# jingsenzhu/i2-sdf

Measured on AMD Instinct MI355X. Metric: ray-samples/sec (fwd+bwd), higher is better.
Workload: dtype f32 (bf16x3 split MFMA: fp32 operands as 3 bf16 terms, fp32 accumulate; the 256x256 weight-gradient GEMM blocks and the sampler's depth-choosing sdf-only passes: 2 bf16 terms per operand, 3 products, fp32 accumulate; the saved SDF tensors abar / G(hbar) / G(a) -- operands of those GEMMs and of the s

## Files before the change

### i2sdf_amd/csrc/mlp_args.h

```cpp
#pragma once
#include "mlp_common.h"

struct SdfTrainFwdArgs {
  const float* fwd; int n_fwd;
  const float* rev; int n_rev;
  int L, skip;
  i2sdf::PointSpec pts;
  int64_t M, Mp;
  float* sdf;
  float* feat;
  float* grad;
  float* hs;
  float* abars;
  float* pe_save;
  int kcs = 16;
  int p24 = 0;
  int wg0 = 0;
  int64_t ldf = 0;
};

struct SdfBwdArgs {
  const float* fwd; int n_fwd;
  const float* rev; int n_rev;
  int L, skip;
// ... 11 lines not shown
  int kcs = 16;
  int p24 = 0;
  int wg0 = 0;
};

struct RgbFwdArgs {
  const float* fwd; int n_fwd; int L;
  const float* dirs; int n_per_ray;
  const float* feat;
  int64_t M, Mp;
  float* rgb;
  float* rs;
  float* pev_save;
  int kcs = 16;
  int wg0 = 0;
};

struct RgbBwdArgs {
  const float* rev; int n_rev; int L;
  int64_t M, Mp;
  const float* rgb;
  const float* rgb_bar;
  const float* rs;
  float* gar;
  float* ga_last;
  float* fbar;
  int kcs = 16;
  int wg0 = 0;
};

void i2sdf_launch_igrad3(const SdfTrainFwdArgs& a, unsigned grid, hipStream_t st);
void i2sdf_launch_sdf_bwd3(const SdfBwdArgs& a, unsigned grid, hipStream_t st);
void i2sdf_launch_train_fwd3h(const SdfTrainFwdArgs& a, unsigned grid, hipStream_t st);
void i2sdf_launch_rgb_fwd3h(const RgbFwdArgs& a, unsigned grid, hipStream_t st);
void i2sdf_launch_rgb_bwd3h(const RgbBwdArgs& a, unsigned grid, hipStream_t st);
struct LightFwd3hArgs {
  const float* fwd; int n_fwd;
  const float* feat;
  int64_t M;
  float* lm;
  float* hl;
};
void i2sdf_launch_light_fwd3h(const LightFwd3hArgs& a, unsigned grid, hipStream_t st);
// ... 1 lines not shown
```

### i2sdf_amd/csrc/mlp_bwd.hip

```cpp
#include "ksplit.h"
#include "mlp_args.h"

using namespace i2sdf;

int i2sdf_hip_check(hipError_t e, const char* what);


namespace {

template <int H, int F, int LF>
__global__ __launch_bounds__(256) void sdf_bwd_kernel(SdfBwdArgs a) {
  constexpr int NT = H / 32, KC = H / 8, PEC = PE<LF>::PEC, PT = cdiv(PEC * 8, 32), FC = F / 8;
  extern __shared__ __attribute__((aligned(16))) float lds[];
  const int tid = threadIdx.x, lane = tid & 63, wave = tid >> 6, hi = lane >> 5;
  const int64_t m = ((int64_t)(blockIdx.x + a.wg0) * 4 + wave) * 32 + (lane & 31);
  const bool valid = m < a.M;
  const int64_t mc = valid ? m : a.M - 1;
  const int64_t lstride = a.Mp * H;
  float gp[PEC * 4];
  {
    float px, py, pz, full[PEC * 8], coef[PEC * 8], nb[3] = {0.f, 0.f, 0.f};
    fetch_point(a.pts, mc, px, py, pz);
    pe_full<LF>(px, py, pz, full);
    pe_coef<LF>(full, coef);
// ... 347 lines not shown
    auto full = [&](hipStream_t s, int wg0, unsigned g, int64_t Mv) {
      SdfBwdArgs x = x3 ? a3 : a;
      x.wg0 = wg0; x.M = Mv;
      if (x3) i2sdf_launch_sdf_bwd3(x, g, s);
      else launch_lds(sdf_bwd_kernel<256, 256, 6>, g, s, x);
    };
    i2sdf_dispatch_points(p, st, M, ranged, true, TAIL_FORKED, full, tail);
  } else if (p->H == 64 && p->F == 64) {
    launch_lds(sdf_bwd_kernel<64, 64, 6>, (unsigned)((M + PTS_PER_WG - 1) / PTS_PER_WG), st, a);
  } else return I2SDF_EINVAL;
  return i2sdf_hip_check(hipGetLastError(), "sdf_backward launch");
}

extern "C" int i2sdf_rgb_backward(const i2sdf_plan* p, const float* packed, const float* rgb, const float* rgb_bar, const float* rs,
                                  int64_t M, int64_t Mp, float* gar, float* ga_last, float* fbar, void* stream) {
  if (M == 0) return I2SDF_OK;
  if (!p || !packed || !rgb || !rgb_bar || !rs || !gar || !ga_last || !fbar || M < 0) return I2SDF_EINVAL;
  if (Mp < M || Mp % PTS_PER_WG) return I2SDF_EINVAL;
  const i2sdf_mlp_desc& d = p->rgb.d;
  const bool wide = d.hidden == 256 && p->F == 256, x3 = wide && p->rgb_bf16x3;
  if (!wide && !(d.hidden == 64 && p->F == 64)) return I2SDF_EINVAL;
  const Span rev = span(p, packed, p->rgb, SPAN_REV);
  if (!rev.n_stages) return I2SDF_EINVAL;
  RgbBwdArgs a{};
  a.rev = rev.w; a.n_rev = rev.n_stages;
  a.L = d.n_lin; a.M = M; a.Mp = Mp; a.rgb = rgb; a.rgb_bar = rgb_bar; a.rs = rs; a.gar = gar; a.ga_last = ga_last; a.fbar = fbar;
  RgbBwdArgs a3 = a;
  if (x3) {
    const Span rev3 = span(p, packed, p->rgb, SPAN_REV3H);
    if (!rev3.n_stages) return I2SDF_EINVAL;
    a3.rev = rev3.w; a3.n_rev = rev3.n_stages;
    a3.kcs = rgb_blocked_points(p, M, Mp) > 0 ? KCS_BLK : KCS_PM;
  }
  hipStream_t st = (hipStream_t)stream;
  const bool ranged = x3 && i2sdf_parts_on(p);
  ChainGuard guard(p, st, ranged);
  auto full = [&](hipStream_t s, int wg0, unsigned g, int64_t Mv) {
    RgbBwdArgs x = x3 ? a3 : a;
    x.wg0 = wg0; x.M = Mv;
    if (x3) i2sdf_launch_rgb_bwd3h(x, g, s);
    else launch_lds(rgb_bwd_kernel<256, 256>, g, s, x);
  };
  auto tail = [&](hipStream_t s, int64_t m0) {
    launch_lds_bytes(KS_LDS_BYTES, rgb_bwd_split_kernel<256, 256>, (unsigned)((M - m0 + 31) / 32), s, a, m0);
  };
  if (wide) i2sdf_dispatch_points(p, st, M, ranged, true, TAIL_BEHIND, full, tail);
  else launch_lds(rgb_bwd_kernel<64, 64>, (unsigned)((M + PTS_PER_WG - 1) / PTS_PER_WG), st, a);
// ... 3 lines not shown
```

### i2sdf_amd/csrc/mlp_train.hip

```cpp
#include "ksplit.h"
#include "mlp_args.h"

using namespace i2sdf;

int i2sdf_hip_check(hipError_t e, const char* what);


namespace {

template <int H, int F, int LF, bool GRAD>
__global__ __launch_bounds__(256) void sdf_train_fwd_kernel(SdfTrainFwdArgs a) {
  constexpr int NT = H / 32, KC = H / 8, PEC = PE<LF>::PEC, PT = cdiv(PEC * 8, 32), FT = F / 32;
  extern __shared__ __attribute__((aligned(16))) float lds[];
  const int tid = threadIdx.x, lane = tid & 63, wave = tid >> 6, hi = lane >> 5;
  const int64_t m = ((int64_t)(blockIdx.x + a.wg0) * 4 + wave) * 32 + (lane & 31);
  const bool valid = m < a.M;
  const int64_t mc = valid ? m : a.M - 1;
  float px, py, pz;
  fetch_point(a.pts, mc, px, py, pz);
  float pe[PEC * 4];
  {
    float full[PEC * 8];
    pe_full<LF>(px, py, pz, full);
    to_b_layout<PEC>(full, pe, hi);
// ... 353 lines not shown
      if (grad) i2sdf_launch_igrad3(x, g, s);
    } else if (wide) {
      if (grad) launch_lds(sdf_train_fwd_kernel<256, 256, 6, true>, g, s, x);
      else launch_lds(sdf_train_fwd_kernel<256, 256, 6, false>, g, s, x);
    } else {
      if (grad) launch_lds(sdf_train_fwd_kernel<64, 64, 6, true>, g, s, x);
      else launch_lds(sdf_train_fwd_kernel<64, 64, 6, false>, g, s, x);
    }
  };
  i2sdf_dispatch_points(p, st, M, ranged, wide && feat != nullptr, TAIL_FORKED, full, tail);
  return i2sdf_hip_check(hipGetLastError(), "sdf_forward_grad launch");
}

extern "C" int i2sdf_rgb_forward(const i2sdf_plan* p, const float* packed, const float* dirs, int32_t n_per_ray, const float* feat,
                                 int64_t M, int64_t Mp, float* rgb, float* rs, float* pev_save, void* stream) {
  if (M == 0) return I2SDF_OK;
  if (!p || !packed || !dirs || !feat || !rgb || M < 0 || n_per_ray <= 0) return I2SDF_EINVAL;
  if (Mp < M || Mp % PTS_PER_WG) return I2SDF_EINVAL;
  const i2sdf_mlp_desc& d = p->rgb.d;
  if (d.multires != 4) return I2SDF_EINVAL;
  const bool wide = d.hidden == 256 && p->F == 256, x3 = wide && p->rgb_bf16x3;
  if (!wide && !(d.hidden == 64 && p->F == 64)) return I2SDF_EINVAL;
  const Span fwd = span(p, packed, p->rgb, SPAN_FWD);
  if (!fwd.n_stages) return I2SDF_EINVAL;
  RgbFwdArgs a{};
  a.fwd = fwd.w; a.n_fwd = fwd.n_stages;
  a.L = d.n_lin; a.dirs = dirs; a.n_per_ray = n_per_ray; a.feat = feat; a.M = M; a.Mp = Mp; a.rgb = rgb; a.rs = rs; a.pev_save = pev_save;
  RgbFwdArgs a3 = a;
  if (x3) {
    const Span fwd3 = span(p, packed, p->rgb, SPAN_FWD3H);
    if (!fwd3.n_stages) return I2SDF_EINVAL;
    a3.fwd = fwd3.w; a3.n_fwd = fwd3.n_stages;
    a3.kcs = rgb_blocked_points(p, M, Mp) > 0 ? KCS_BLK : KCS_PM;
  }
  hipStream_t st = (hipStream_t)stream;
  const bool ranged = x3 && i2sdf_parts_on(p);
  ChainGuard guard(p, st, ranged);
  auto full = [&](hipStream_t s, int wg0, unsigned g, int64_t Mv) {
    RgbFwdArgs x = x3 ? a3 : a;
    x.wg0 = wg0; x.M = Mv;
    if (x3) i2sdf_launch_rgb_fwd3h(x, g, s);
    else launch_lds(rgb_fwd_kernel<256, 256, 4>, g, s, x);
  };
  auto tail = [&](hipStream_t s, int64_t m0) {
    launch_lds_bytes(KS_LDS_BYTES, rgb_fwd_split_kernel<256, 256, 4>, (unsigned)((M - m0 + 31) / 32), s, a, m0);
  };
  if (wide) i2sdf_dispatch_points(p, st, M, ranged, true, TAIL_BEHIND, full, tail);
  else launch_lds(rgb_fwd_kernel<64, 64, 4>, (unsigned)((M + PTS_PER_WG - 1) / PTS_PER_WG), st, a);
// ... 112 lines not shown
```

### i2sdf_amd/csrc/mlp_x3h.hip

```cpp
#define I2SDF_RELU_ASM 1
#include "mlp_args.h"
#include "x3h.h"

using namespace i2sdf;

namespace {

template <int LF>
__device__ __forceinline__ void pe_select_h(float px, float py, float pz, float (&pe)[cdiv(PE<LF>::DIM, 32) * 8], int kg) {
  constexpr int PED = PE<LF>::DIM, PE32 = cdiv(PED, 32);
  float full[PE<LF>::PEC * 8], pad[PE32 * 32];
  pe_full<LF>(px, py, pz, full);
#pragma unroll
  for (int i = 0; i < PE32 * 32; ++i) pad[i] = (i < PED) ? full[i < PE<LF>::PEC * 8 ? i : 0] : 0.f;
  x3h_select<PE32>(pad, pe, kg);
}

template <int H, int LF, int NW, int PL>
__global__ __launch_bounds__(NW * 64, 2) void sdf_fwd3h_kernel(const float* __restrict__ stream, int n_stages, int L, int skip, PointSpec ps,
                                                                const int* __restrict__ skip_flag, int64_t M, float* __restrict__ sdf_out) {
  constexpr int NT = H / 16, KH32 = H / 32, PE32 = cdiv(PE<LF>::DIM, 32), NPE = PE32 * 8;
  extern __shared__ __attribute__((aligned(16))) float lds[];
  if (skip_flag != nullptr && skip_flag[0] != 0) return;
  const int tid = threadIdx.x, lane = tid & 63, wave = tid >> 6, kg = lane >> 4;
// ... 77 lines not shown
#pragma unroll
    for (int r = 0; r < 4; ++r) h[nt * 4 + r] = softplus100(accA[nt][r]);
  if (a.hs) store_regs_h<NT>(a.hs + (a.L - 2) * lstride + mrow, kg, valid, h, kcs);
  {
    float s[1];
    rowvec_h<1, NT, NW>(ws, h, s, tid);
    if (a.sdf != nullptr && valid && kg == 0) a.sdf[m] = s[0];
  }
  if (a.feat != nullptr) {
    XhRegSrc<NT * 4> src{h};
    dense_x3h<FT, KH32, 1, NW>(ws, src, accB, tid);
    store_tile_h<FT>(a.feat + mc * (a.ldf ? a.ldf : (int64_t)F), kg, valid, accB);
  }
}

template <int H, int F, int LFV, int NW>
__global__ __launch_bounds__(NW * 64, 2) void rgb_fwd3h_kernel(RgbFwdArgs a) {
  constexpr int NT = H / 16, KH32 = H / 32, PECV = PE<LFV>::PEC, PV32 = cdiv(PE<LFV>::DIM, 32);
  extern __shared__ __attribute__((aligned(16))) float lds[];
  const int tid = threadIdx.x, lane = tid & 63, wave = tid >> 6, kg = lane >> 4;
  const int64_t m = ((int64_t)(blockIdx.x + a.wg0) * NW + wave) * HP + (lane & 15);
  const bool valid = m < a.M;
  const int64_t mc = valid ? m : a.M - 1;
  const int64_t ray = mc / a.n_per_ray;
  float pev[PV32 * 8];
  pe_select_h<LFV>(a.dirs[ray * 3 + 0], a.dirs[ray * 3 + 1], a.dirs[ray * 3 + 2], pev, kg);
  if (a.pev_save) store_pe_row_h<PECV>(a.pev_save + m * (PECV * 8), kg, valid, pev);
  const int64_t lstride = a.Mp * H;
  const int kcs = a.kcs;
  const int64_t mrow = save_row_off(m, kcs);
  WStreamH<NW> ws;
  ws.begin(a.fwd, lds, a.n_fwd, tid);
  f32x4 accA[NT], accB[NT];
  {
    XhPeRowSrc<PV32> src{pev, a.feat + mc * F, kg};
    dense_x3h<NT, PV32 + F / 32, 1, NW>(ws, src, accA, tid);
  }
  for (int l = 1; l < a.L - 1; ++l) {
    XhReluSrc<NT> src{accA, a.rs ? a.rs + (l - 1) * lstride + mrow : nullptr, kg, valid, kcs};
    dense_x3h<NT, KH32, 1, NW>(ws, src, accB, tid);
#pragma unroll
    for (int nt = 0; nt < NT; ++nt) accA[nt] = accB[nt];
  }
  float r[NT * 4];
#pragma unroll
  for (int nt = 0; nt < NT; ++nt)
#pragma unroll
    for (int q = 0; q < 4; ++q) r[nt * 4 + q] = fmaxf(accA[nt][q], 0.f);
  if (a.rs) store_regs_h<NT>(a.rs + (a.L - 2) * lstride + mrow, kg, valid, r, kcs);
  float o[3];
  rowvec_h<3, NT, NW>(ws, r, o, tid);
  if (valid && kg == 0) {
#pragma unroll
    for (int i = 0; i < 3; ++i) a.rgb[m * 3 + i] = 1.0f / (1.0f + expf(-o[i]));
  }
}

template <int HL, int F, int NW>
__global__ __launch_bounds__(NW * 64, 2) void light_fwd3h_kernel(LightFwd3hArgs a) {
  constexpr int NT = HL / 16, KF32 = F / 32;
  extern __shared__ __attribute__((aligned(16))) float lds[];
  const int tid = threadIdx.x, lane = tid & 63, wave = tid >> 6, kg = lane >> 4;
  const int64_t m = ((int64_t)blockIdx.x * NW + wave) * HP + (lane & 15);
  const bool valid = m < a.M;
// ... 4 lines not shown
  {
    XhRowSrc<true> src{a.feat + mc * F, kg};
    dense_x3h<NT, KF32, 1, NW>(ws, src, acc, tid);
  }
  float h[NT * 4];
#pragma unroll
  for (int nt = 0; nt < NT; ++nt)
#pragma unroll
    for (int r = 0; r < 4; ++r) h[nt * 4 + r] = softplus100(acc[nt][r]);
  if (a.hl) store_regs_h<NT>(a.hl + m * HL, kg, valid, h, 16);
  float o[1];
  rowvec_h<1, NT, NW>(ws, h, o, tid);
  if (valid && kg == 0) a.lm[m] = 1.0f / (1.0f + expf(-o[0]));
}

template <int H, int F, int NW>
__global__ __launch_bounds__(NW * 64, 2) void rgb_bwd3h_kernel(RgbBwdArgs a) {
  constexpr int NT = H / 16, KH32 = H / 32, FT = F / 16;
  static_assert(FT == NT, "feature tiles reuse the hidden accumulator set");
  extern __shared__ __attribute__((aligned(16))) float lds[];
  const int tid = threadIdx.x, lane = tid & 63, wave = tid >> 6, kg = lane >> 4;
  const int64_t m = ((int64_t)(blockIdx.x + a.wg0) * NW + wave) * HP + (lane & 15);
  const bool valid = m < a.M;
  const int64_t mc = valid ? m : a.M - 1;
  const int64_t lstride = a.Mp * H;
  const int kcs = a.kcs;
  const int64_t mrow = save_row_off(m, kcs), mcrow = save_row_off(mc, kcs);
  float g3[3];
#pragma unroll
  for (int j = 0; j < 3; ++j) {
    const float c = a.rgb[mc * 3 + j];
    g3[j] = a.rgb_bar[mc * 3 + j] * c * (1.0f - c);
  }
  if (valid && kg == 0) *reinterpret_cast<f32x4*>(a.ga_last + m * 4) = f32x4{g3[0], g3[1], g3[2], 0.f};
  WStreamH<NW> ws;
  ws.begin(a.rev, lds, a.n_rev, tid);
  float ga[NT * 4];
  {
    constexpr int NWC = 3 * NT, TOT = rowvec_h_chunks(NT, 3), NS = TOT / SCH;
#pragma unroll
    for (int i = 0; i < NT * 4; ++i) ga[i] = 0.f;
#pragma unroll
    for (int s = 0; s < NS; ++s) {
      const f32x4* cur = reinterpret_cast<const f32x4*>(ws.advance(tid)) + lane;
#pragma unroll
      for (int j = 0; j < SCH; ++j) {
        const int c = s * SCH + j;
        if (c < NWC) {
          const int row = c / NT, nt = c % NT;
          const f32x4 w = cur[j * 64];
          ga[nt * 4 + 0] = fmaf(w.x, g3[row], ga[nt * 4 + 0]);
          ga[nt * 4 + 1] = fmaf(w.y, g3[row], ga[nt * 4 + 1]);
          ga[nt * 4 + 2] = fmaf(w.z, g3[row], ga[nt * 4 + 2]);
          ga[nt * 4 + 3] = fmaf(w.w, g3[row], ga[nt * 4 + 3]);
        }
      }
    }
    const int l = a.L - 2;
    const float* rrow = a.rs + l * lstride + mcrow;
    float* grow = a.gar + l * lstride + mrow;
#pragma unroll
    for (int nt = 0; nt < NT; ++nt) {
      const f32x4 rv = *reinterpret_cast<const f32x4*>(rrow + nt * kcs + 4 * kg);
      f32x4 o;
#pragma unroll
      for (int t = 0; t < 4; ++t) { o[t] = rv[t] > 0.f ? ga[nt * 4 + t] : 0.f; ga[nt * 4 + t] = o[t]; }
      if (valid) *reinterpret_cast<f32x4*>(grow + nt * kcs + 4 * kg) = o;
    }
  }
  f32x4 accA[NT], accB[NT];
  auto zero = [&](f32x4 (&x)[NT]) __attribute__((always_inline)) {
#pragma unroll
    for (int nt = 0; nt < NT; ++nt) x[nt] = f32x4{0.f, 0.f, 0.f, 0.f};
  };
  {
    XhRegSrc<NT * 4> src{ga};
    zero(accA);
    dense_x3h<NT, KH32, 0, NW>(ws, src, accA, tid);
  }
  for (int l = a.L - 3; l >= 1; --l) {
    XhMaskSrc<NT> src{accA, a.rs + l * lstride + mcrow, a.gar + l * lstride + mrow, kg, valid, kcs};
    zero(accB);
    dense_x3h<NT, KH32, 0, NW>(ws, src, accB, tid);
#pragma unroll
    for (int nt = 0; nt < NT; ++nt) accA[nt] = accB[nt];
  }
  {
    XhMaskSrc<NT> src{accA, a.rs + mcrow, a.gar + mrow, kg, valid, kcs};
    zero(accB);
    dense_x3h<FT, KH32, 0, NW>(ws, src, accB, tid);
    store_tile_h<FT>(a.fbar + mc * F, kg, valid, accB);
  }
}

}

void i2sdf_launch_sdf_fwd3h(const float* stream, int n_stages, int L, int skip, const PointSpec& ps, const int* skip_flag, int64_t M, float* sdf_out,
                            int planes, hipStream_t st) {
  const unsigned grid = (unsigned)((M + 8 * HP - 1) / (8 * HP));
  if (planes == 2) launch_lds_threads(512, sdf_fwd3h_kernel<256, 6, 8, 2>, grid, st, stream, n_stages, L, skip, ps, skip_flag, M, sdf_out);
  else launch_lds_threads(512, sdf_fwd3h_kernel<256, 6, 8, 3>, grid, st, stream, n_stages, L, skip, ps, skip_flag, M, sdf_out);
}
void i2sdf_launch_train_fwd3h(const SdfTrainFwdArgs& a, unsigned grid, hipStream_t st) { launch_lds_threads(512, sdf_train_fwd3h_kernel<256, 256, 6, 8>, grid, st, a); }
void i2sdf_launch_rgb_fwd3h(const RgbFwdArgs& a, unsigned grid, hipStream_t st) { launch_lds_threads(512, rgb_fwd3h_kernel<256, 256, 4, 8>, grid, st, a); }
void i2sdf_launch_light_fwd3h(const LightFwd3hArgs& a, unsigned grid, hipStream_t st) { launch_lds_threads(8 * 64, light_fwd3h_kernel<128, 256, 8>, grid, st, a); }
void i2sdf_launch_rgb_bwd3h(const RgbBwdArgs& a, unsigned grid, hipStream_t st) { launch_lds_threads(512, rgb_bwd3h_kernel<256, 256, 8>, grid, st, a); }
```

### i2sdf_amd/csrc/x3h.h

```cpp
#pragma once
#include "x3.h"

namespace i2sdf {

constexpr int HP = 16;
constexpr int XH_AHEAD = 1, XH_RING = XH_AHEAD + 1;
constexpr int SCH = SC;
constexpr int LDS_BYTES_H = LDS_BYTES;
template <int NW> using WStreamH = WStreamT<NW * 64, SCH>;

__host__ __device__ constexpr int x3h_op_chunks(int NT, int KC32, int PL = 3) { return round_up(NT + KC32 * NT * PL, SCH); }
__host__ __device__ constexpr int x3h_bwd_chunks(int KT, int KC32) { return round_up(KC32 * KT * 3, SCH); }
__host__ __device__ constexpr int rowvec_h_chunks(int NTK, int nrows) { return round_up(nrows * NTK + 1, SCH); }

__device__ __forceinline__ f32x4 mfma_bf16h(u32x4 a, u32x4 b, f32x4 c) {
  return __builtin_amdgcn_mfma_f32_16x16x32_bf16(__builtin_bit_cast(bf16x8, a), __builtin_bit_cast(bf16x8, b), c, 0, 0, 0);
}

template <int NC32>
__device__ __forceinline__ void x3h_select(const float (&full)[NC32 * 32], float (&sel)[NC32 * 8], int kg) {
  const unsigned m1 = (kg & 1) ? 0xffffffffu : 0u, m2 = (kg & 2) ? 0xffffffffu : 0u;
  auto pick = [](unsigned m, float a, float b) __attribute__((always_inline)) {
    return __builtin_bit_cast(float, (__builtin_bit_cast(unsigned, a) & m) | (__builtin_bit_cast(unsigned, b) & ~m));
  };
// ... 204 lines not shown
    if (kc < KACC && hrow != nullptr && valid) x3h_store8(hrow, kc, kg, v, kcs);
    return 0;
  }
};
template <int NREG>
struct XhRegSrc {
  static constexpr bool STORES = false;
  const float (&r)[NREG];
  __device__ __forceinline__ int ahead(int) { return 0; }
  __device__ __forceinline__ float p1(int, int) { return 0.f; }
  __device__ __forceinline__ float p2(int, int, float) { return 0.f; }
  __device__ __forceinline__ float p3(int kc, int u, float, float, float&) { return r[8 * kc + u]; }
  __device__ __forceinline__ int done(int, const float (&)[8], const float (&)[8]) { return 0; }
};

template <int NT>
struct XhReluSrc {
  static constexpr bool STORES = true;
  const f32x4 (&accP)[NT]; float* rrow; int kg; bool valid; int kcs = 16;
  __device__ __forceinline__ int ahead(int) { return 0; }
  __device__ __forceinline__ float p1(int, int) { return 0.f; }
  __device__ __forceinline__ float p2(int, int, float) { return 0.f; }
  __device__ __forceinline__ float p3(int kc, int u, float, float, float&) { return relu0(accP[2 * kc + (u >> 2)][u & 3]); }
  __device__ __forceinline__ int done(int kc, const float (&v)[8], const float (&)[8]) {
    if (rrow != nullptr && valid) x3h_store8(rrow, kc, kg, v, kcs);
    return 0;
  }
};
template <int NPV>
struct XhPeRowSrc {
  static constexpr bool STORES = false;
  const float (&pe)[NPV * 8]; const float* row; int kg;
  f32x4 q[XH_RING][2];
  __device__ __forceinline__ int ahead(int kc) { if (kc >= NPV) x3h_load8(row, kc - NPV, kg, q[kc % XH_RING], 16); return kc >= NPV ? 2 : 0; }
  __device__ __forceinline__ float p1(int, int) { return 0.f; }
  __device__ __forceinline__ float p2(int, int, float) { return 0.f; }
  __device__ __forceinline__ float p3(int kc, int u, float, float, float&) { return kc < NPV ? pe[8 * (kc < NPV ? kc : 0) + u] : q[kc % XH_RING][u >> 2][u & 3]; }
  __device__ __forceinline__ int done(int, const float (&)[8], const float (&)[8]) { return 0; }
// ... 14 lines not shown
};
template <int NT>
struct XhMaskSrc {
  static constexpr bool STORES = true;
  const f32x4 (&accP)[NT]; const float* rrow; float* grow; int kg; bool valid; int kcs = 16;
  f32x4 q[XH_RING][2];
  __device__ __forceinline__ int ahead(int kc) { x3h_load8(rrow, kc, kg, q[kc % XH_RING], kcs); return 2; }
  __device__ __forceinline__ float p1(int, int) { return 0.f; }
  __device__ __forceinline__ float p2(int, int, float) { return 0.f; }
  __device__ __forceinline__ float p3(int kc, int u, float, float, float&) { return q[kc % XH_RING][u >> 2][u & 3] > 0.f ? accP[2 * kc + (u >> 2)][u & 3] : 0.f; }
  __device__ __forceinline__ int done(int kc, const float (&v)[8], const float (&)[8]) {
    x3h_store8(grow, kc, kg, v, kcs);
    return X3_COUNT_STORES ? 2 : 0;
  }
};

template <int NTK>
__device__ __forceinline__ void store_regs_h(float* __restrict__ row, int kg, bool valid, const float (&r)[NTK * 4], int kcs) {
  if (!valid) return;
#pragma unroll
  for (int nt = 0; nt < NTK; ++nt) stg4(row + nt * kcs + 4 * kg, f32x4{r[4 * nt], r[4 * nt + 1], r[4 * nt + 2], r[4 * nt + 3]});
}
template <int NTK>
__device__ __forceinline__ void store_tile_h(float* __restrict__ row, int kg, bool valid, const f32x4 (&t)[NTK]) {
  if (!valid) return;
#pragma unroll
  for (int nt = 0; nt < NTK; ++nt) stg4(row + 16 * nt + 4 * kg, t[nt]);
}
}
```

### i2sdf_amd/engine.py

```python
from __future__ import annotations

import ctypes as C
from typing import Optional

import os

import torch

from . import lib as L
from .config import NetConfig
from .params import ParamLayout


class RenderEngine:
    def __init__(self, cfg: NetConfig, device="cuda"):
        self.cfg = cfg
        self.layout = ParamLayout(cfg)
        self.device = torch.device(device)
        self._lib = L.load()
        self._desc = self.layout.net_desc()
        plan = C.c_void_p()
        L.check(self._lib.i2sdf_plan_create(C.byref(self._desc), C.byref(plan)), "i2sdf_plan_create")
        self._plan = plan
        self.pack_floats = int(self._lib.i2sdf_plan_pack_floats(plan))
        self.wgrad_floats = int(self._lib.i2sdf_plan_wgrad_floats(plan))
        self.packed = torch.zeros(self.pack_floats, dtype=torch.float32, device=self.device)
        self._pack_stream, self._pack_event, self._pack_readers = None, None, {}
        self.F = cfg.feature_size
        wide = cfg.sdf.hidden == 256 and cfg.feature_size == 256
        self.set_sdf_forward_bf16x3(bool(cfg.bf16x3 and cfg.sdf.hidden % 64 == 0))
        self.set_wgrad_bf16x3(bool(cfg.bf16x3))
        self.set_train_forward_bf16x3(bool(cfg.bf16x3 and wide))
        self.set_sdf_backward_bf16x3(bool(cfg.bf16x3 and wide))
        self.set_rgb_bf16x3(bool(cfg.bf16x3 and cfg.rgb.hidden == 256 and cfg.feature_size == 256 and cfg.rgb.n_lin >= 3))
        self.wgrad_bf16x2 = False
        x2 = os.environ.get("I2SDF_WGRAD_BF16X2", "")
        self.set_wgrad_bf16x2(bool(cfg.bf16x3 and ((x2 != "0") if x2 != "" else cfg.wgrad_bf16x2)))
        self.sampler_bf16x2 = False
        sx2 = os.environ.get("I2SDF_SAMPLER_BF16X2", "")
        if wide:
            self.set_sampler_bf16x2(bool(self.sdf_forward_bf16x3 and ((sx2 != "0") if sx2 != "" else getattr(cfg, "sampler_bf16x2", False))))
        self.set_blocked_saves(bool(cfg.bf16x3 and os.environ.get("I2SDF_BLOCKED_SAVES", "1") != "0"))
        self.saves24 = False
        s24 = os.environ.get("I2SDF_SAVES24", "")
        if wide:
            self.set_saves24(bool(cfg.bf16x3 and ((s24 != "0") if s24 != "" else getattr(cfg, "saves24", True))))
        self.set_tail_overlap(os.environ.get("I2SDF_TAIL_OVERLAP", "1") != "0")
        self.parts = 0
        n_parts = int(os.environ.get("I2SDF_PARTS", "2"))
# ... 7 lines not shown
        self.u_more = torch.linspace(0.0, 1.0, steps=sc.N_samples_eval, device=dev)
        self.u_final = torch.linspace(0.0, 1.0, steps=sc.N_samples, device=dev)
        if sc.N_samples_extra > 0:
            self.extra_tab = torch.stack([torch.linspace(0, sc.N_samples_eval * (it + 1) - 1, sc.N_samples_extra).long()
                                          for it in range(sc.max_total_iters)]).to(torch.int32).to(dev).contiguous()
        else:
            self.extra_tab = None
        self.n_z = sc.N_samples + sc.N_samples_extra + 2

    def start_timing(self):
        self._timing = []
        eng = self

        class _Timed:
            def __init__(self, fn, name):
                self.fn, self.name = fn, name

            def __call__(self, *a):
                e0, e1 = torch.cuda.Event(enable_timing=True), torch.cuda.Event(enable_timing=True)
                e0.record()
                rc = self.fn(*a)
                e1.record()
                eng._timing.append((self.name, e0, e1))
                return rc

        self._timed_lib = type("TimedLib", (), {})()
        for name in L.SIGNATURES:
            fn = getattr(self._lib, name)
            if name in ("i2sdf_sdf_forward", "i2sdf_sdf_forward_grad", "i2sdf_rgb_forward", "i2sdf_rgb_backward", "i2sdf_sdf_backward",
                        "i2sdf_weight_grads", "i2sdf_sample_rays", "i2sdf_composite_forward", "i2sdf_composite_backward", "i2sdf_pack_weights",
                        "i2sdf_ray_setup", "i2sdf_light_forward", "i2sdf_light_backward"):
                fn = _Timed(fn, name)
            setattr(self._timed_lib, name, fn)
        self._real_lib, self._lib = self._lib, self._timed_lib

    def stop_timing(self):
        self._lib = self._real_lib
        out = {}
        for name, e0, e1 in self._timing:
            tot, cnt = out.get(name, (0.0, 0))
            out[name] = (tot + e0.elapsed_time(e1), cnt + 1)
        self._timing = []
        return out

# ... 105 lines not shown
                out[l] = v.reshape(Mp, 256)
        return out

    def saved_pm(self, name: str, t: torch.Tensor, M: int, has_feat: bool = True) -> torch.Tensor:
        Mp = t.shape[1]
        if name in ("rs", "gar"):
            return self.saved_to_point_major(t, self.blocked_points(1, M, Mp))[:, :M]
        nb = self.blocked_points(0, M, Mp, has_feat)
        p24 = None
        if name in ("abars", "gus", "gas") and self.saves24_points(M, Mp, has_feat) == Mp:
            p24 = [True] * t.shape[0]
            if name == "gus":
                p24[-1] = False
                p24[0] = False
        return self.saved_to_point_major(t, nb, p24)[:, :M]

    def set_tail_overlap(self, on: bool):
        L.check(self._lib.i2sdf_plan_set_option(self._plan, L.OPT_TAIL_OVERLAP, int(bool(on))), "i2sdf_plan_set_option")
        self.tail_overlap = bool(on)

    def _sync_parts(self):
        want = self._parts_wanted if (self.train_forward_bf16x3 and self.sdf_backward_bf16x3 and self.rgb_bf16x3) else 0
        if want != self.parts:
            n = int(want) if int(want) >= 2 else 0
            L.check(self._lib.i2sdf_plan_set_option(self._plan, L.OPT_PARTS, n), "i2sdf_plan_set_option")
            self.parts = n

    def set_parts(self, n: int):
        self._parts_wanted = int(n) if int(n) >= 2 else 0
        self._sync_parts()
# ... 64 lines not shown
        out["hs"] = self._ws(NL - 1, Mp, H, device=dev) if (save or want_grad) else None
        out["abars"] = self._ws(NL - 1, Mp, H, device=dev) if (save and want_grad) else None
        out["pe"] = self._ws(Mp, 40, device=dev) if save else None
        L.check(self._lib.i2sdf_sdf_forward_grad(self._plan, self._pk(), L.ptr(pts), L.ptr(cam), L.ptr(dirs), L.ptr(z),
                                                  ldz, npr, n_ray, M, Mp, L.ptr(out["sdf"]), L.ptr(out["feat"]), L.ptr(out["grad"]),
                                                  L.ptr(out["hs"]), L.ptr(out["abars"]), L.ptr(out["pe"]), L.stream_ptr()),
                 "i2sdf_sdf_forward_grad")
        return out

    def rgb_forward(self, dirs, n_per_ray, feat, M, save=True):
        Mp = feat.shape[0]
        rgb = torch.empty(M, 3, dtype=torch.float32, device=feat.device)
        Lr, Hr = self.cfg.rgb.n_lin, self.cfg.rgb.hidden
        rs = self._ws(Lr - 1, Mp, Hr, device=feat.device) if save else None
        pev = self._ws(Mp, 32, device=feat.device) if save else None
        L.check(self._lib.i2sdf_rgb_forward(self._plan, self._pk(), L.ptr(dirs.contiguous()), n_per_ray, L.ptr(feat), M, Mp,
                                             L.ptr(rgb), L.ptr(rs), L.ptr(pev), L.stream_ptr()), "i2sdf_rgb_forward")
        return rgb, rs, pev

    def rgb_backward(self, rgb, rgb_bar, rs, M):
        Mp, dev = rs.shape[1], rs.device
        Lr, Hr = self.cfg.rgb.n_lin, self.cfg.rgb.hidden
        gar = self._ws(Lr - 1, Mp, Hr, device=dev)
        ga_last = self._ws(Mp, 4, device=dev)
        fbar = self._ws(Mp, self.F, device=dev)
        L.check(self._lib.i2sdf_rgb_backward(self._plan, self._pk(), L.ptr(rgb), L.ptr(rgb_bar.contiguous()), L.ptr(rs), M, Mp,
                                              L.ptr(gar), L.ptr(ga_last), L.ptr(fbar), L.stream_ptr()), "i2sdf_rgb_backward")
        return gar, ga_last, fbar

    def sdf_backward(self, fw, sbar=None, fbar=None, m_fbar=0, nbar=None):
        cfgs = self.cfg.sdf
        H, NL = cfgs.hidden, cfgs.n_lin
        Mp, M, dev = fw["Mp"], fw["M"], fw["hs"].device
        cam, dirs, z, npr = fw["rays"]
        o = {"gus": self._ws(NL, Mp, H, device=dev), "gpbar": self._ws(Mp, 40, device=dev), "gas": self._ws(NL - 1, Mp, H, device=dev),
             "ga_last4": self._ws(Mp, 4, device=dev), "ones4": self._ws(Mp, 4, device=dev)}
        c = lambda t: None if t is None else t.contiguous()
        L.check(self._lib.i2sdf_sdf_backward(self._plan, self._pk(), L.ptr(fw["pts"]), L.ptr(cam), L.ptr(dirs), L.ptr(z),
                                              z.shape[1] if z is not None else 0, npr, fw["n_ray_pts"], M, Mp,
                                              L.ptr(fw["hs"]), L.ptr(fw["abars"]), L.ptr(c(sbar)), L.ptr(c(fbar)), m_fbar, L.ptr(c(nbar)),
                                              L.ptr(o["gus"]), L.ptr(o["gpbar"]), L.ptr(o["gas"]), L.ptr(o["ga_last4"]), L.ptr(o["ones4"]),
                                              L.stream_ptr()), "i2sdf_sdf_backward")
# ... 200 lines not shown
```

### i2sdf_amd/lib.py

```python
from __future__ import annotations

import ctypes as C
import os

MAX_LAYERS = 12
_HERE = os.path.dirname(os.path.abspath(__file__))
LIB_PATH = os.environ.get("I2SDF_LIB_PATH") or os.path.join(_HERE, "lib", "libi2sdf_hip.so")


class MlpDesc(C.Structure):
    _fields_ = [("n_lin", C.c_int32), ("hidden", C.c_int32), ("d_in", C.c_int32), ("in0", C.c_int32), ("d_out", C.c_int32),
                ("multires", C.c_int32), ("skip_layer", C.c_int32), ("reserved", C.c_int32),
                ("out_dim", C.c_int32 * MAX_LAYERS), ("in_dim", C.c_int32 * MAX_LAYERS),
                ("off_bias", C.c_int64 * MAX_LAYERS), ("off_g", C.c_int64 * MAX_LAYERS), ("off_v", C.c_int64 * MAX_LAYERS)]


class NetDesc(C.Structure):
    _fields_ = [("sdf", MlpDesc), ("rgb", MlpDesc), ("light", MlpDesc), ("off_beta", C.c_int64), ("n_params", C.c_int64),
                ("beta_min", C.c_float), ("scene_bounding_sphere", C.c_float)]


class TrainBuffers(C.Structure):
    _fields_ = [("M_sdf", C.c_int64), ("M_main", C.c_int64), ("Mp", C.c_int64)] + [(n, C.c_void_p) for n in (
        "pe", "hs", "abars", "gus", "gpbar", "gas", "ga_last4", "ones4", "fbar", "pev", "feat", "rs", "gar", "ga_last_rgb",
# ... 66 lines not shown
    "i2sdf_last_hip_error": (C.c_char_p, []),
    "i2sdf_plan_create": (C.c_int, [C.POINTER(NetDesc), C.POINTER(_P)]),
    "i2sdf_plan_destroy": (None, [_P]),
    "i2sdf_plan_set_option": (C.c_int, [_P, _I32, _I32]),
    "i2sdf_chain_begin": (C.c_int, [_P, _I64, _P]),
    "i2sdf_chain_fence": (C.c_int, [_P, _P]),
    "i2sdf_chain_end": (C.c_int, [_P, _P]),
    "i2sdf_blocked_points": (_I64, [_P, _I32, _I64, _I64, _I32]),
    "i2sdf_plan_pack_floats": (_I64, [_P]),
    "i2sdf_plan_wgrad_floats": (_I64, [_P]),
    "i2sdf_pack_weights": (C.c_int, [_P, _P, _P, _P]),
    "i2sdf_sdf_forward": (C.c_int, [_P, _P, _P, _I64, _P, _P, _I64, _P]),
    "i2sdf_sdf_forward_grad": (C.c_int, [_P] * 6 + [_I64, _I32, _I64, _I64, _I64] + [_P] * 7),
    "i2sdf_rgb_forward": (C.c_int, [_P, _P, _P, _I32, _P, _I64, _I64, _P, _P, _P, _P]),
    "i2sdf_rgb_backward": (C.c_int, [_P] * 5 + [_I64, _I64] + [_P] * 4),
    "i2sdf_sdf_backward": (C.c_int, [_P] * 6 + [_I64, _I32, _I64, _I64, _I64] + [_P] * 4 + [_I64] + [_P] * 7),
    "i2sdf_wgrad_chunk_points": (_I64, []),
    "i2sdf_weight_grads": (C.c_int, [_P, C.POINTER(TrainBuffers), _P, _P, _I64, _P, _P]),
    "i2sdf_comm_available": (_I32, []),
    "i2sdf_comm_unique_id": (C.c_int, [_P, _I64]),
    "i2sdf_comm_init_rank": (C.c_int, [_P, _I32, _I32, C.POINTER(_P)]),
    "i2sdf_comm_destroy": (None, [_P]),
    "i2sdf_comm_size": (_I32, [_P]),
    "i2sdf_comm_rank": (_I32, [_P]),
    "i2sdf_last_comm_error": (C.c_char_p, []),
    "i2sdf_allreduce_grads": (C.c_int, [_P, _I64, _P, _P]),
    "i2sdf_allreduce_max_i32": (C.c_int, [_P, _I64, _P, _P]),
    "i2sdf_broadcast": (C.c_int, [_P, _I64, _I32, _P, _P]),
    "i2sdf_comm_as_exchange": (C.c_int, [_P, C.POINTER(Exchange)]),
    "i2sdf_plan_set_exchange": (C.c_int, [_P, C.POINTER(Exchange), _I32]),
# ... 108 lines not shown
```

### include/i2sdf.h

```cpp
#ifndef I2SDF_H
#define I2SDF_H

#include <stddef.h>
#include <stdint.h>

#ifdef __cplusplus
extern "C" {
#endif

#define I2SDF_VERSION 100
#define I2SDF_MAX_LAYERS 12
#define I2SDF_MAX_PARTS 4

#define I2SDF_OK 0
#define I2SDF_EINVAL (-1)
#define I2SDF_EHIP (-2)
#define I2SDF_ESPHERE (-3)
#define I2SDF_EWORKSPACE (-4)
#define I2SDF_ECOMM (-5)

typedef struct i2sdf_mlp_desc {
  int32_t n_lin;
  int32_t hidden;
  int32_t d_in;
// ... 47 lines not shown
int64_t i2sdf_plan_wgrad_floats(const i2sdf_plan* plan);

int i2sdf_pack_weights(const i2sdf_plan* plan, const float* params, float* packed, void* stream);

int i2sdf_sdf_forward(const i2sdf_plan* plan, const float* packed, const float* points, int64_t M,
                      float* sdf_out, float* feat_out, int64_t ld_feat, void* stream);


int i2sdf_sdf_forward_grad(const i2sdf_plan* plan, const float* packed, const float* points, const float* cam,
                           const float* dirs, const float* z, int64_t ldz, int32_t n_per_ray, int64_t n_ray_pts, int64_t M,
                           int64_t Mp, float* sdf, float* feat, float* grad, float* hs, float* abars, float* pe_save,
                           void* stream);

int i2sdf_rgb_forward(const i2sdf_plan* plan, const float* packed, const float* dirs, int32_t n_per_ray, const float* feat,
                      int64_t M, int64_t Mp, float* rgb, float* rs, float* pev_save, void* stream);

int i2sdf_rgb_backward(const i2sdf_plan* plan, const float* packed, const float* rgb, const float* rgb_bar, const float* rs,
                       int64_t M, int64_t Mp, float* gar, float* ga_last, float* fbar, void* stream);

int i2sdf_sdf_backward(const i2sdf_plan* plan, const float* packed, const float* points, const float* cam, const float* dirs,
                       const float* z, int64_t ldz, int32_t n_per_ray, int64_t n_ray_pts, int64_t M, int64_t Mp,
                       const float* hs, const float* abars, const float* sbar, const float* fbar, int64_t m_fbar,
                       const float* nbar, float* gus, float* gpbar, float* gas, float* ga_last4, float* ones4, void* stream);

int i2sdf_ray_setup(const float* uv, const float* pose, const float* intrinsics, int64_t batch, int32_t pixels,
                    float* cam_loc, float* dirs, float* dnorm, void* stream);
int i2sdf_ray_setup_ex(const float* uv, const float* pose, int32_t pose_is_quat, const float* intrinsics, int64_t batch,
                       int32_t pixels, float* cam_loc, float* dirs, float* dnorm, void* stream);

typedef struct i2sdf_ray_tables {
  const float* intrinsics;
  const float* pose;
  int32_t pose_is_quat;
// ... 258 lines not shown
```

Baseline: 21.01 million.

## Save packed ReLU bitmasks in rgb forward and use them in rgb backward

Result: no change. 20.89 million (-0.6%).

```diff
diff --git a/i2sdf_amd/csrc/mlp_args.h b/i2sdf_amd/csrc/mlp_args.h
--- a/i2sdf_amd/csrc/mlp_args.h
+++ b/i2sdf_amd/csrc/mlp_args.h
@@ -49,6 +49,7 @@
   float* pev_save;
   int kcs = 16;
   int wg0 = 0;
+  uint32_t* rmask = nullptr;
 };
 
 struct RgbBwdArgs {
@@ -62,6 +63,7 @@
   float* fbar;
   int kcs = 16;
   int wg0 = 0;
+  const uint32_t* rmask = nullptr;
 };
 
 void i2sdf_launch_igrad3(const SdfTrainFwdArgs& a, unsigned grid, hipStream_t st);
diff --git a/i2sdf_amd/csrc/mlp_bwd.hip b/i2sdf_amd/csrc/mlp_bwd.hip
--- a/i2sdf_amd/csrc/mlp_bwd.hip
+++ b/i2sdf_amd/csrc/mlp_bwd.hip
@@ -385,6 +385,11 @@
 
 extern "C" int i2sdf_rgb_backward(const i2sdf_plan* p, const float* packed, const float* rgb, const float* rgb_bar, const float* rs,
                                   int64_t M, int64_t Mp, float* gar, float* ga_last, float* fbar, void* stream) {
+  return i2sdf_rgb_backward_m(p, packed, rgb, rgb_bar, rs, nullptr, M, Mp, gar, ga_last, fbar, stream);
+}
+
+extern "C" int i2sdf_rgb_backward_m(const i2sdf_plan* p, const float* packed, const float* rgb, const float* rgb_bar, const float* rs,
+                                    const uint32_t* rmask, int64_t M, int64_t Mp, float* gar, float* ga_last, float* fbar, void* stream) {
   if (M == 0) return I2SDF_OK;
   if (!p || !packed || !rgb || !rgb_bar || !rs || !gar || !ga_last || !fbar || M < 0) return I2SDF_EINVAL;
   if (Mp < M || Mp % PTS_PER_WG) return I2SDF_EINVAL;
@@ -402,6 +407,7 @@
     if (!rev3.n_stages) return I2SDF_EINVAL;
     a3.rev = rev3.w; a3.n_rev = rev3.n_stages;
     a3.kcs = rgb_blocked_points(p, M, Mp) > 0 ? KCS_BLK : KCS_PM;
+    a3.rmask = rmask;
   }
   hipStream_t st = (hipStream_t)stream;
   const bool ranged = x3 && i2sdf_parts_on(p);
diff --git a/i2sdf_amd/csrc/mlp_train.hip b/i2sdf_amd/csrc/mlp_train.hip
--- a/i2sdf_amd/csrc/mlp_train.hip
+++ b/i2sdf_amd/csrc/mlp_train.hip
@@ -391,6 +391,11 @@
 
 extern "C" int i2sdf_rgb_forward(const i2sdf_plan* p, const float* packed, const float* dirs, int32_t n_per_ray, const float* feat,
                                  int64_t M, int64_t Mp, float* rgb, float* rs, float* pev_save, void* stream) {
+  return i2sdf_rgb_forward_m(p, packed, dirs, n_per_ray, feat, M, Mp, rgb, rs, nullptr, pev_save, stream);
+}
+
+extern "C" int i2sdf_rgb_forward_m(const i2sdf_plan* p, const float* packed, const float* dirs, int32_t n_per_ray, const float* feat,
+                                   int64_t M, int64_t Mp, float* rgb, float* rs, uint32_t* rmask, float* pev_save, void* stream) {
   if (M == 0) return I2SDF_OK;
   if (!p || !packed || !dirs || !feat || !rgb || M < 0 || n_per_ray <= 0) return I2SDF_EINVAL;
   if (Mp < M || Mp % PTS_PER_WG) return I2SDF_EINVAL;
@@ -409,6 +414,7 @@
     if (!fwd3.n_stages) return I2SDF_EINVAL;
     a3.fwd = fwd3.w; a3.n_fwd = fwd3.n_stages;
     a3.kcs = rgb_blocked_points(p, M, Mp) > 0 ? KCS_BLK : KCS_PM;
+    a3.rmask = rmask;
   }
   hipStream_t st = (hipStream_t)stream;
   const bool ranged = x3 && i2sdf_parts_on(p);
diff --git a/i2sdf_amd/csrc/mlp_x3h.hip b/i2sdf_amd/csrc/mlp_x3h.hip
--- a/i2sdf_amd/csrc/mlp_x3h.hip
+++ b/i2sdf_amd/csrc/mlp_x3h.hip
@@ -115,7 +115,7 @@
   }
 }
 
-template <int H, int F, int LFV, int NW>
+template <int H, int F, int LFV, int NW, bool MASK>
 __global__ __launch_bounds__(NW * 64, 2) void rgb_fwd3h_kernel(RgbFwdArgs a) {
   constexpr int NT = H / 16, KH32 = H / 32, PECV = PE<LFV>::PEC, PV32 = cdiv(PE<LFV>::DIM, 32);
   extern __shared__ __attribute__((aligned(16))) float lds[];
@@ -138,8 +138,10 @@
     dense_x3h<NT, PV32 + F / 32, 1, NW>(ws, src, accA, tid);
   }
   for (int l = 1; l < a.L - 1; ++l) {
-    XhReluSrc<NT> src{accA, a.rs ? a.rs + (l - 1) * lstride + mrow : nullptr, kg, valid, kcs};
+    XhReluSrc<NT, MASK> src{accA, a.rs ? a.rs + (l - 1) * lstride + mrow : nullptr, kg, valid, kcs};
     dense_x3h<NT, KH32, 1, NW>(ws, src, accB, tid);
+    if (MASK && valid)
+      *reinterpret_cast<uint2*>(a.rmask + x3h_mask_off(l - 1, a.Mp, m, kg)) = uint2{x3h_mask_word(src.mk[0]), x3h_mask_word(src.mk[1])};
 #pragma unroll
     for (int nt = 0; nt < NT; ++nt) accA[nt] = accB[nt];
   }
@@ -149,6 +151,13 @@
 #pragma unroll
     for (int q = 0; q < 4; ++q) r[nt * 4 + q] = fmaxf(accA[nt][q], 0.f);
   if (a.rs) store_regs_h<NT>(a.rs + (a.L - 2) * lstride + mrow, kg, valid, r, kcs);
+  if (MASK) {
+    static_assert(!MASK || NT * 4 == 64, "two mask words per lane and layer");
+    unsigned mk[2] = {0u, 0u};
+#pragma unroll
+    for (int i = 0; i < NT * 4; ++i) x3h_push_gt0(mk[i >> 5], r[i]);
+    if (valid) *reinterpret_cast<uint2*>(a.rmask + x3h_mask_off(a.L - 2, a.Mp, m, kg)) = uint2{x3h_mask_word(mk[0]), x3h_mask_word(mk[1])};
+  }
   float o[3];
   rowvec_h<3, NT, NW>(ws, r, o, tid);
   if (valid && kg == 0) {
@@ -183,7 +192,7 @@
   if (valid && kg == 0) a.lm[m] = 1.0f / (1.0f + expf(-o[0]));
 }
 
-template <int H, int F, int NW>
+template <int H, int F, int NW, bool BITS>
 __global__ __launch_bounds__(NW * 64, 2) void rgb_bwd3h_kernel(RgbBwdArgs a) {
   constexpr int NT = H / 16, KH32 = H / 32, FT = F / 16;
   static_assert(FT == NT, "feature tiles reuse the hidden accumulator set");
@@ -202,6 +211,13 @@
     g3[j] = a.rgb_bar[mc * 3 + j] * c * (1.0f - c);
   }
   if (valid && kg == 0) *reinterpret_cast<f32x4*>(a.ga_last + m * 4) = f32x4{g3[0], g3[1], g3[2], 0.f};
+  static_assert(!BITS || NT * 4 == 64, "two mask words per lane and layer");
+  const uint2* mrow2 = BITS ? reinterpret_cast<const uint2*>(a.rmask + x3h_mask_off(0, a.Mp, mc, kg)) : nullptr;
+  uint2 mtop = {0u, 0u}, mnext = {0u, 0u};
+  if (BITS) {
+    mtop = mrow2[(a.L - 2) * a.Mp * 4];
+    mnext = mrow2[(a.L >= 3 ? a.L - 3 : 0) * a.Mp * 4];
+  }
   WStreamH<NW> ws;
   ws.begin(a.rev, lds, a.n_rev, tid);
   float ga[NT * 4];
@@ -230,10 +246,15 @@
     float* grow = a.gar + l * lstride + mrow;
 #pragma unroll
     for (int nt = 0; nt < NT; ++nt) {
-      const f32x4 rv = *reinterpret_cast<const f32x4*>(rrow + nt * kcs + 4 * kg);
       f32x4 o;
-#pragma unroll
-      for (int t = 0; t < 4; ++t) { o[t] = rv[t] > 0.f ? ga[nt * 4 + t] : 0.f; ga[nt * 4 + t] = o[t]; }
+      if (BITS) {
+#pragma unroll
+        for (int t = 0; t < 4; ++t) { o[t] = x3h_mask_sel(mtop.x, mtop.y, nt * 4 + t, ga[nt * 4 + t]); ga[nt * 4 + t] = o[t]; }
+      } else {
+        const f32x4 rv = *reinterpret_cast<const f32x4*>(rrow + nt * kcs + 4 * kg);
+#pragma unroll
+        for (int t = 0; t < 4; ++t) { o[t] = rv[t] > 0.f ? ga[nt * 4 + t] : 0.f; ga[nt * 4 + t] = o[t]; }
+      }
       if (valid) *reinterpret_cast<f32x4*>(grow + nt * kcs + 4 * kg) = o;
     }
   }
@@ -248,16 +269,28 @@
     dense_x3h<NT, KH32, 0, NW>(ws, src, accA, tid);
   }
   for (int l = a.L - 3; l >= 1; --l) {
-    XhMaskSrc<NT> src{accA, a.rs + l * lstride + mcrow, a.gar + l * lstride + mrow, kg, valid, kcs};
     zero(accB);
-    dense_x3h<NT, KH32, 0, NW>(ws, src, accB, tid);
+    if constexpr (BITS) {
+      const uint2 mcur = mnext;
+      mnext = mrow2[(l - 1) * a.Mp * 4];
+      XhBitSrc<NT> src{accA, mcur.x, mcur.y, a.gar + l * lstride + mrow, kg, valid, kcs};
+      dense_x3h<NT, KH32, 0, NW>(ws, src, accB, tid);
+    } else {
+      XhMaskSrc<NT> src{accA, a.rs + l * lstride + mcrow, a.gar + l * lstride + mrow, kg, valid, kcs};
+      dense_x3h<NT, KH32, 0, NW>(ws, src, accB, tid);
+    }
 #pragma unroll
     for (int nt = 0; nt < NT; ++nt) accA[nt] = accB[nt];
   }
   {
-    XhMaskSrc<NT> src{accA, a.rs + mcrow, a.gar + mrow, kg, valid, kcs};
     zero(accB);
-    dense_x3h<FT, KH32, 0, NW>(ws, src, accB, tid);
+    if constexpr (BITS) {
+      XhBitSrc<NT> src{accA, mnext.x, mnext.y, a.gar + mrow, kg, valid, kcs};
+      dense_x3h<FT, KH32, 0, NW>(ws, src, accB, tid);
+    } else {
+      XhMaskSrc<NT> src{accA, a.rs + mcrow, a.gar + mrow, kg, valid, kcs};
+      dense_x3h<FT, KH32, 0, NW>(ws, src, accB, tid);
+    }
     store_tile_h<FT>(a.fbar + mc * F, kg, valid, accB);
   }
 }
@@ -271,6 +304,12 @@
   else launch_lds_threads(512, sdf_fwd3h_kernel<256, 6, 8, 3>, grid, st, stream, n_stages, L, skip, ps, skip_flag, M, sdf_out);
 }
 void i2sdf_launch_train_fwd3h(const SdfTrainFwdArgs& a, unsigned grid, hipStream_t st) { launch_lds_threads(512, sdf_train_fwd3h_kernel<256, 256, 6, 8>, grid, st, a); }
-void i2sdf_launch_rgb_fwd3h(const RgbFwdArgs& a, unsigned grid, hipStream_t st) { launch_lds_threads(512, rgb_fwd3h_kernel<256, 256, 4, 8>, grid, st, a); }
+void i2sdf_launch_rgb_fwd3h(const RgbFwdArgs& a, unsigned grid, hipStream_t st) {
+  if (a.rmask != nullptr) launch_lds_threads(512, rgb_fwd3h_kernel<256, 256, 4, 8, true>, grid, st, a);
+  else launch_lds_threads(512, rgb_fwd3h_kernel<256, 256, 4, 8, false>, grid, st, a);
+}
 void i2sdf_launch_light_fwd3h(const LightFwd3hArgs& a, unsigned grid, hipStream_t st) { launch_lds_threads(8 * 64, light_fwd3h_kernel<128, 256, 8>, grid, st, a); }
-void i2sdf_launch_rgb_bwd3h(const RgbBwdArgs& a, unsigned grid, hipStream_t st) { launch_lds_threads(512, rgb_bwd3h_kernel<256, 256, 8>, grid, st, a); }
+void i2sdf_launch_rgb_bwd3h(const RgbBwdArgs& a, unsigned grid, hipStream_t st) {
+  if (a.rmask != nullptr) launch_lds_threads(512, rgb_bwd3h_kernel<256, 256, 8, true>, grid, st, a);
+  else launch_lds_threads(512, rgb_bwd3h_kernel<256, 256, 8, false>, grid, st, a);
+}
diff --git a/i2sdf_amd/csrc/x3h.h b/i2sdf_amd/csrc/x3h.h
--- a/i2sdf_amd/csrc/x3h.h
+++ b/i2sdf_amd/csrc/x3h.h
@@ -242,14 +242,42 @@
   __device__ __forceinline__ int done(int, const float (&)[8], const float (&)[8]) { return 0; }
 };
 
-template <int NT>
+__device__ __forceinline__ void x3h_push_gt0(unsigned& m, float v) {
+  asm("v_cmp_lt_f32 vcc, 0, %1\n\tv_addc_co_u32 %0, vcc, %0, %0, vcc" : "+v"(m) : "v"(v) : "vcc");
+}
+__device__ __forceinline__ unsigned x3h_mask_word(unsigned pushed) { return __builtin_bitreverse32(pushed); }
+__device__ __forceinline__ int64_t x3h_mask_off(int slot, int64_t Mp, int64_t m, int kg) { return ((slot * Mp + m) * 4 + kg) * 2; }
+template <int B> __device__ __forceinline__ unsigned x3h_sbit(unsigned w) {
+  unsigned s;
+  asm("v_bfe_i32 %0, %1, %2, 1" : "=v"(s) : "v"(w), "n"(B));
+  return s;
+}
+__device__ __forceinline__ float x3h_mask_sel(unsigned w0, unsigned w1, int b, float acc) {
+  const unsigned w = b < 32 ? w0 : w1;
+  unsigned s = 0u;
+  switch (b & 31) {
+#define X3H_SB(i) case i: s = x3h_sbit<i>(w); break;
+    X3H_SB(0) X3H_SB(1) X3H_SB(2) X3H_SB(3) X3H_SB(4) X3H_SB(5) X3H_SB(6) X3H_SB(7) X3H_SB(8) X3H_SB(9) X3H_SB(10) X3H_SB(11) X3H_SB(12) X3H_SB(13)
+    X3H_SB(14) X3H_SB(15) X3H_SB(16) X3H_SB(17) X3H_SB(18) X3H_SB(19) X3H_SB(20) X3H_SB(21) X3H_SB(22) X3H_SB(23) X3H_SB(24) X3H_SB(25) X3H_SB(26)
+    X3H_SB(27) X3H_SB(28) X3H_SB(29) X3H_SB(30) X3H_SB(31)
+#undef X3H_SB
+  }
+  return __builtin_bit_cast(float, __builtin_bit_cast(unsigned, acc) & s);
+}
+
+template <int NT, bool MASK = false>
 struct XhReluSrc {
   static constexpr bool STORES = true;
   const f32x4 (&accP)[NT]; float* rrow; int kg; bool valid; int kcs = 16;
+  unsigned mk[2] = {0u, 0u};
   __device__ __forceinline__ int ahead(int) { return 0; }
   __device__ __forceinline__ float p1(int, int) { return 0.f; }
   __device__ __forceinline__ float p2(int, int, float) { return 0.f; }
-  __device__ __forceinline__ float p3(int kc, int u, float, float, float&) { return relu0(accP[2 * kc + (u >> 2)][u & 3]); }
+  __device__ __forceinline__ float p3(int kc, int u, float, float, float&) {
+    const float r = relu0(accP[2 * kc + (u >> 2)][u & 3]);
+    if (MASK) x3h_push_gt0(mk[kc >> 2], r);
+    return r;
+  }
   __device__ __forceinline__ int done(int kc, const float (&v)[8], const float (&)[8]) {
     if (rrow != nullptr && valid) x3h_store8(rrow, kc, kg, v, kcs);
     return 0;
@@ -294,6 +322,19 @@
     return X3_COUNT_STORES ? 2 : 0;
   }
 };
+template <int NT>
+struct XhBitSrc {
+  static constexpr bool STORES = true;
+  const f32x4 (&accP)[NT]; unsigned w0, w1; float* grow; int kg; bool valid; int kcs = 16;
+  __device__ __forceinline__ int ahead(int) { return 0; }
+  __device__ __forceinline__ float p1(int, int) { return 0.f; }
+  __device__ __forceinline__ float p2(int, int, float) { return 0.f; }
+  __device__ __forceinline__ float p3(int kc, int u, float, float, float&) { return x3h_mask_sel(w0, w1, 8 * kc + u, accP[2 * kc + (u >> 2)][u & 3]); }
+  __device__ __forceinline__ int done(int kc, const float (&v)[8], const float (&)[8]) {
+    x3h_store8(grow, kc, kg, v, kcs);
+    return X3_COUNT_STORES ? 2 : 0;
+  }
+};
 
 template <int NTK>
 __device__ __forceinline__ void store_regs_h(float* __restrict__ row, int kg, bool valid, const float (&r)[NTK * 4], int kcs) {
diff --git a/i2sdf_amd/engine.py b/i2sdf_amd/engine.py
--- a/i2sdf_amd/engine.py
+++ b/i2sdf_amd/engine.py
@@ -33,6 +33,8 @@
         self.set_train_forward_bf16x3(bool(cfg.bf16x3 and wide))
         self.set_sdf_backward_bf16x3(bool(cfg.bf16x3 and wide))
         self.set_rgb_bf16x3(bool(cfg.bf16x3 and cfg.rgb.hidden == 256 and cfg.feature_size == 256 and cfg.rgb.n_lin >= 3))
+        self.rgb_mask = os.environ.get("I2SDF_RGB_MASK", "1") != "0"
+        self.rgb_mask_used, self.rgb_mask_unused = 0, 0
         self.wgrad_bf16x2 = False
         x2 = os.environ.get("I2SDF_WGRAD_BF16X2", "")
         self.set_wgrad_bf16x2(bool(cfg.bf16x3 and ((x2 != "0") if x2 != "" else cfg.wgrad_bf16x2)))
@@ -70,7 +72,7 @@
 
         class _Timed:
             def __init__(self, fn, name):
-                self.fn, self.name = fn, name
+                self.fn, self.name = fn, {"i2sdf_rgb_forward_m": "i2sdf_rgb_forward", "i2sdf_rgb_backward_m": "i2sdf_rgb_backward"}.get(name, name)
 
             def __call__(self, *a):
                 e0, e1 = torch.cuda.Event(enable_timing=True), torch.cuda.Event(enable_timing=True)
@@ -84,6 +86,7 @@
         for name in L.SIGNATURES:
             fn = getattr(self._lib, name)
             if name in ("i2sdf_sdf_forward", "i2sdf_sdf_forward_grad", "i2sdf_rgb_forward", "i2sdf_rgb_backward", "i2sdf_sdf_backward",
+                        "i2sdf_rgb_forward_m", "i2sdf_rgb_backward_m",
                         "i2sdf_weight_grads", "i2sdf_sample_rays", "i2sdf_composite_forward", "i2sdf_composite_backward", "i2sdf_pack_weights",
                         "i2sdf_ray_setup", "i2sdf_light_forward", "i2sdf_light_backward"):
                 fn = _Timed(fn, name)
@@ -219,6 +222,17 @@
                 p24[-1] = False
                 p24[0] = False
         return self.saved_to_point_major(t, nb, p24)[:, :M]
+
+    def set_rgb_mask(self, on: bool):
+        self.rgb_mask = bool(on)
+
+    @staticmethod
+    def saved_mask(mask: torch.Tensor, M: int) -> torch.Tensor:
+        Lr, Mp = mask.shape[0], mask.shape[1]
+        w = mask.contiguous().view(torch.int32).reshape(Lr, Mp, 4, 2)[:, :M].to(torch.int64) & 0xFFFFFFFF
+        sh = torch.arange(32, device=mask.device, dtype=torch.int64)
+        bits = ((w.unsqueeze(-1) >> sh) & 1).bool().reshape(Lr, M, 4, 8, 2, 4)
+        return bits.permute(0, 1, 3, 4, 2, 5).reshape(Lr, M, 256)
 
     def set_tail_overlap(self, on: bool):
         L.check(self._lib.i2sdf_plan_set_option(self._plan, L.OPT_TAIL_OVERLAP, int(bool(on))), "i2sdf_plan_set_option")
@@ -313,9 +327,21 @@
         Lr, Hr = self.cfg.rgb.n_lin, self.cfg.rgb.hidden
         rs = self._ws(Lr - 1, Mp, Hr, device=feat.device) if save else None
         pev = self._ws(Mp, 32, device=feat.device) if save else None
-        L.check(self._lib.i2sdf_rgb_forward(self._plan, self._pk(), L.ptr(dirs.contiguous()), n_per_ray, L.ptr(feat), M, Mp,
-                                             L.ptr(rgb), L.ptr(rs), L.ptr(pev), L.stream_ptr()), "i2sdf_rgb_forward")
+        mask = self._ws(Lr - 1, Mp, 8, device=feat.device) if (save and self.rgb_mask and self.rgb_bf16x3 and Hr == 256) else None
+        L.check(self._lib.i2sdf_rgb_forward_m(self._plan, self._pk(), L.ptr(dirs.contiguous()), n_per_ray, L.ptr(feat), M, Mp,
+                                               L.ptr(rgb), L.ptr(rs), L.ptr(mask), L.ptr(pev), L.stream_ptr()), "i2sdf_rgb_forward")
+        if mask is not None:
+            rs._i2sdf_rmask = (mask, rs._version, self._rgb_mask_key(M))
         return rgb, rs, pev
+
+    def _rgb_mask_key(self, M):
+        return (int(M), bool(self.rgb_bf16x3), int(self.parts), bool(self.blocked_saves))
+
+    def _rgb_mask_of(self, rs, M):
+        tag = getattr(rs, "_i2sdf_rmask", None) if self.rgb_mask else None
+        if tag is None or tag[1] != rs._version or tag[2] != self._rgb_mask_key(M) or tag[0].shape[1] != rs.shape[1]:
+            return None
+        return tag[0]
 
     def rgb_backward(self, rgb, rgb_bar, rs, M):
         Mp, dev = rs.shape[1], rs.device
@@ -323,8 +349,13 @@
         gar = self._ws(Lr - 1, Mp, Hr, device=dev)
         ga_last = self._ws(Mp, 4, device=dev)
         fbar = self._ws(Mp, self.F, device=dev)
-        L.check(self._lib.i2sdf_rgb_backward(self._plan, self._pk(), L.ptr(rgb), L.ptr(rgb_bar.contiguous()), L.ptr(rs), M, Mp,
-                                              L.ptr(gar), L.ptr(ga_last), L.ptr(fbar), L.stream_ptr()), "i2sdf_rgb_backward")
+        mask = self._rgb_mask_of(rs, M)
+        if mask is not None:
+            self.rgb_mask_used += 1
+        else:
+            self.rgb_mask_unused += 1
+        L.check(self._lib.i2sdf_rgb_backward_m(self._plan, self._pk(), L.ptr(rgb), L.ptr(rgb_bar.contiguous()), L.ptr(rs), L.ptr(mask), M, Mp,
+                                                L.ptr(gar), L.ptr(ga_last), L.ptr(fbar), L.stream_ptr()), "i2sdf_rgb_backward")
         return gar, ga_last, fbar
 
     def sdf_backward(self, fw, sbar=None, fbar=None, m_fbar=0, nbar=None):
diff --git a/i2sdf_amd/lib.py b/i2sdf_amd/lib.py
--- a/i2sdf_amd/lib.py
+++ b/i2sdf_amd/lib.py
@@ -104,6 +104,8 @@
     "i2sdf_sdf_forward_grad": (C.c_int, [_P] * 6 + [_I64, _I32, _I64, _I64, _I64] + [_P] * 7),
     "i2sdf_rgb_forward": (C.c_int, [_P, _P, _P, _I32, _P, _I64, _I64, _P, _P, _P, _P]),
     "i2sdf_rgb_backward": (C.c_int, [_P] * 5 + [_I64, _I64] + [_P] * 4),
+    "i2sdf_rgb_forward_m": (C.c_int, [_P, _P, _P, _I32, _P, _I64, _I64, _P, _P, _P, _P, _P]),
+    "i2sdf_rgb_backward_m": (C.c_int, [_P] * 6 + [_I64, _I64] + [_P] * 4),
     "i2sdf_sdf_backward": (C.c_int, [_P] * 6 + [_I64, _I32, _I64, _I64, _I64] + [_P] * 4 + [_I64] + [_P] * 7),
     "i2sdf_wgrad_chunk_points": (_I64, []),
     "i2sdf_weight_grads": (C.c_int, [_P, C.POINTER(TrainBuffers), _P, _P, _I64, _P, _P]),
diff --git a/include/i2sdf.h b/include/i2sdf.h
--- a/include/i2sdf.h
+++ b/include/i2sdf.h
@@ -85,9 +85,13 @@
 
 int i2sdf_rgb_forward(const i2sdf_plan* plan, const float* packed, const float* dirs, int32_t n_per_ray, const float* feat,
                       int64_t M, int64_t Mp, float* rgb, float* rs, float* pev_save, void* stream);
+int i2sdf_rgb_forward_m(const i2sdf_plan* plan, const float* packed, const float* dirs, int32_t n_per_ray, const float* feat,
+                        int64_t M, int64_t Mp, float* rgb, float* rs, uint32_t* rmask, float* pev_save, void* stream);
 
 int i2sdf_rgb_backward(const i2sdf_plan* plan, const float* packed, const float* rgb, const float* rgb_bar, const float* rs,
                        int64_t M, int64_t Mp, float* gar, float* ga_last, float* fbar, void* stream);
+int i2sdf_rgb_backward_m(const i2sdf_plan* plan, const float* packed, const float* rgb, const float* rgb_bar, const float* rs,
+                         const uint32_t* rmask, int64_t M, int64_t Mp, float* gar, float* ga_last, float* fbar, void* stream);
 
 int i2sdf_sdf_backward(const i2sdf_plan* plan, const float* packed, const float* points, const float* cam, const float* dirs,
                        const float* z, int64_t ldz, int32_t n_per_ray, int64_t n_ray_pts, int64_t M, int64_t Mp,
```
